# orybkin/video-gcp

Hardware: AMD Instinct MI355X
Metric: predicted frames/sec, 64x64x3 seq_len=80 gcp_tree (posterior forward + all loss terms, model(inputs) and model.loss() of train.py:157-159, batch-stat BatchNorm) (higher is better)
Workload: dtype f32 (encoder / decoder convs and the tree GEMMs from 512 rows: split-f16 MFMA with f32 accumulate, f32-equivalent; everything else exact f32 MFMA)

## Files before the change

### video-gcp_amd/csrc/conv3x3_split.hip

```cpp
#include "common.h"
#include "split_mfma.h"

#include <cstdlib>
#include <type_traits>

namespace {

struct SplitUpCfg {
    static constexpr int RW = 18, RH = 6, LW = 10, LH = 4, CC = 16, KS = 5;
    static constexpr int RAW_BYTES = LH * LW * CC * 4;
    static constexpr int PLANE_BYTES = RH * RW * 32;
    static constexpr int WAVE_BYTES = RAW_BYTES + 2 * PLANE_BYTES;
    static constexpr int NS = (LH * LW * 4 + 63) / 64;
    static constexpr int W_CHUNK_BYTES = KS * 2 * 1024;
    static int lds_bytes(int nchunk) { return nchunk * W_CHUNK_BYTES + 8 * WAVE_BYTES + 8 * 2 * 16 * 4; }
};

__global__ void __launch_bounds__(512, 2) conv3x3_up16_split_kernel(const gcpx_conv_args a, const int items_per_wave,
                                                                    const int nitems) {
    using Cfg = SplitUpCfg;
    constexpr int RW = Cfg::RW, RH = Cfg::RH, LW = Cfg::LW, LH = Cfg::LH, CC = Cfg::CC, NS = Cfg::NS, KS = Cfg::KS;
    extern __shared__ float4 smem4[];
    const int nchunk = a.Cin / CC;
    const char* wl = reinterpret_cast<const char*>(smem4);
// ... 798 lines not shown
    __syncthreads();

    const int c4 = lane & 3, ps = lane >> 2;
    const float* sptr = a.src[0].ptr;
    const int srcC = a.src[0].C;
    float4 bn_s = make_float4(1.f, 1.f, 1.f, 1.f), bn_t = make_float4(0.f, 0.f, 0.f, 0.f);
    if (a.src[0].scale) {
        bn_s = *reinterpret_cast<const float4*>(a.src[0].scale + c4 * 4);
        bn_t = *reinterpret_cast<const float4*>(a.src[0].shift + c4 * 4);
    }
    const float slope = a.src[0].act == GCPX_ACT_LRELU ? 0.2f : 1.f;
    const int fdiv0 = a.src[0].frame_div;
    const int ew = a.w_split_log2_dev ? __builtin_amdgcn_readfirstlane(*a.w_split_log2_dev) : a.w_split_log2;
    const float4 bv = *reinterpret_cast<const float4*>(a.bias + q * 4);

    const int gw = blockIdx.x * 8 + wave;
    int item = gw * items_per_wave;
    const int item_end = min(item + items_per_wave, nitems);
    auto origin = [&](int it, int& f, int& y0, int& x0) {
        const int rb = it % nrb;
        const int t = it / nrb;
        y0 = rb * R; f = t / ncb; x0 = (t % ncb) * 16;
    };
    int p_row[NS], p_col[NS], p_lds[NS];
    bool p_ok[NS];
#pragma unroll
    for (int k = 0; k < NS; ++k) {
        const int pix = ps + 16 * k;
        p_ok[k] = pix < PR * PW;
        p_row[k] = min(pix, PR * PW - 1) / PW;
        p_col[k] = min(pix, PR * PW - 1) % PW;
        p_lds[k] = (p_row[k] * PW + p_col[k]) * 64 + c4 * 16;
    }
    int r_rd[NO], r_wr[NO];
    float r_wa[NO];
    bool r_ok[NO], r_c0[NO], r_c17[NO];
#pragma unroll
    for (int k = 0; k < NO; ++k) {
        const int pix = ps + 16 * k;
        r_ok[k] = pix < PR * RW;
        const int r = min(pix, PR * RW - 1) / RW, c = min(pix, PR * RW - 1) % RW;
        r_rd[k] = (r * PW + (c >> 1)) * 64 + c4 * 16;
        r_wr[k] = (r * RW + c) * 32 + c4 * 8;
        r_wa[k] = (c & 1) ? 0.25f : 0.75f;
        r_c0[k] = c == 0; r_c17[k] = c == RW - 1;
    }
    float4 pre[NS];
    auto issue_loads = [&](int it) {
        int f, y0, x0;
        origin(it, f, y0, x0);
        const float* base = sptr + (size_t)(f / fdiv0) * Hin * Win * srcC + c4 * 4;
        const int ly0 = y0 - 1, lx0 = x0 / 2 - 1;
#pragma unroll
        for (int k = 0; k < NS; ++k) {
            const int sy = min(max(ly0 + p_row[k], 0), Hin - 1), sx = min(max(lx0 + p_col[k], 0), Win - 1);
            pre[k] = *reinterpret_cast<const float4*>(base + (unsigned)((sy * Win + sx) * srcC));
        }
    };

    f32x4 st1 = f32x4{0, 0, 0, 0}, st2 = f32x4{0, 0, 0, 0};
    f32x4 outv[R][2];
    float* optr = nullptr;
    auto store_out = [&]() __attribute__((always_inline)) {
#pragma unroll
        for (int yi = 0; yi < R; ++yi)
#pragma unroll
            for (int py = 0; py < 2; ++py) {
                const f32x4 v = outv[yi][py];
                *reinterpret_cast<float4*>(optr + (unsigned)((2 * yi + py) * W * 16)) = make_float4(v[0], v[1], v[2], v[3]);
            }
    };
    if (item < item_end) issue_loads(item);

    const int boff0 = (j + (q >> 1)) * 32 + (q & 1) * 16, boff1 = (j + 2) * 32 + (q & 1) * 16;

    for (; item < item_end; ++item) {
        int f, y0, x0;
        origin(item, f, y0, x0);
        const bool top = (y0 == 0), bot = (y0 + R == Hin), lft = (x0 == 0), rgt = (x0 + 16 == W);

        float amax = 0.f;
#pragma unroll
        for (int k = 0; k < NS; ++k) {
            float4 v = pre[k];
            v.x = fmaf(v.x, bn_s.x, bn_t.x); v.y = fmaf(v.y, bn_s.y, bn_t.y); v.z = fmaf(v.z, bn_s.z, bn_t.z); v.w = fmaf(v.w, bn_s.w, bn_t.w);
            v.x = fmaxf(v.x, v.x * slope); v.y = fmaxf(v.y, v.y * slope); v.z = fmaxf(v.z, v.z * slope); v.w = fmaxf(v.w, v.w * slope);
            if (p_ok[k]) *reinterpret_cast<float4*>(wbuf + p_lds[k]) = v;
            else v = make_float4(0.f, 0.f, 0.f, 0.f);
            amax = fmaxf(amax, fmaxf(fmaxf(fabsf(v.x), fabsf(v.y)), fmaxf(fabsf(v.z), fabsf(v.w))));
        }
        if (item + 1 < item_end) issue_loads(item + 1);
        if (optr) store_out();
        amax = wave_max_nonneg(amax);
        int ex = 14 + 127 - (int)((__float_as_uint(amax) >> 23) & 0xff);
        ex = __builtin_amdgcn_readfirstlane(amax > 0.f ? max(-100, min(min(100, 126 - ew), ex)) : min(100, 126 - ew));
        const float sx2 = __uint_as_float((unsigned)(127 + ex) << 23);

        h4 o1[NO], o2[NO];
#pragma unroll
        for (int k = 0; k < NO; ++k) {
            const float4 A = *reinterpret_cast<const float4*>(wbuf + r_rd[k]);
            const float4 B = *reinterpret_cast<const float4*>(wbuf + r_rd[k] + 64);
            const float sc = ((lft && r_c0[k]) || (rgt && r_c17[k])) ? 0.f : sx2;
            const float wa = r_wa[k] * sc, wb = (1.f - r_wa[k]) * sc;
            float4 v;
            v.x = fmaf(wa, A.x, wb * B.x); v.y = fmaf(wa, A.y, wb * B.y); v.z = fmaf(wa, A.z, wb * B.z); v.w = fmaf(wa, A.w, wb * B.w);
            h4 p1, p2;
            p1[0] = (_Float16)v.x; p1[1] = (_Float16)v.y; p1[2] = (_Float16)v.z; p1[3] = (_Float16)v.w;
            p2[0] = (_Float16)fmaf((float)p1[0], -1.f, v.x); p2[1] = (_Float16)fmaf((float)p1[1], -1.f, v.y);
            p2[2] = (_Float16)fmaf((float)p1[2], -1.f, v.z); p2[3] = (_Float16)fmaf((float)p1[3], -1.f, v.w);
            o1[k] = p1;
            o2[k] = p2;
        }
        __builtin_amdgcn_fence(__ATOMIC_ACQ_REL, "wavefront");
        __builtin_amdgcn_wave_barrier();
#pragma unroll
        for (int k = 0; k < NO; ++k) {
            if (r_ok[k]) {
                *reinterpret_cast<h4*>(wbuf + r_wr[k]) = o1[k];
                *reinterpret_cast<h4*>(wbuf + r_wr[k] + Cfg::PLANE_BYTES) = o2[k];
            }
        }

        f32x4 acc[R][2];
#pragma unroll
        for (int yi = 0; yi < R; ++yi) { acc[yi][0] = f32x4{0, 0, 0, 0}; acc[yi][1] = f32x4{0, 0, 0, 0}; }
        auto load_w = [&](const int t, h8 (&w)[2]) __attribute__((always_inline)) {
            const char* wp = wl + t * 2048 + lane * 16;
            w[0] = *reinterpret_cast<const h8*>(wp);
            w[1] = *reinterpret_cast<const h8*>(wp + 1024);
        };
        auto load_b = [&](const int kind, const int r, h8 (&b)[2]) __attribute__((always_inline)) {
            const char* bp = wbuf + r * RW * 32 + (kind ? boff1 : boff0);
            b[0] = *reinterpret_cast<const h8*>(bp);
            b[1] = *reinterpret_cast<const h8*>(bp + Cfg::PLANE_BYTES);
        };
        h8 wq[2][2], bq[2][PR][2], wt[2], wb[2];
        load_w(0, wq[0]);
#pragma unroll
        for (int r = 0; r < 4; ++r) load_b(0, r, bq[0][r]);
        __builtin_amdgcn_s_setprio(1);
        static_for<0, 12>([&](auto tc) __attribute__((always_inline)) {
            constexpr int t = decltype(tc)::value, kind = t / 6, blk = t % 6, dyl = blk / 2, py = blk % 2;
// ... 14 lines not shown
#pragma unroll
            for (int yi = 0; yi < R; ++yi) acc[yi][py] = mfma32h(w1, bq[kind & 1][yi + dyl][1], acc[yi][py]);
#pragma unroll
            for (int yi = 0; yi < R; ++yi) acc[yi][py] = mfma32h(w1, bq[kind & 1][yi + dyl][0], acc[yi][py]);
            __builtin_amdgcn_sched_group_barrier(0x100, (more ? 2 : 0) + ((pre_next || pre_own) ? 2 : 0) + (pre_c ? 4 : 0), 0);
            __builtin_amdgcn_sched_group_barrier(0x008, 12, 0);
            if constexpr (blk == 5) {
                if (top) {
                    acc[0][0] = mfma32h(wt[1], bq[kind & 1][0][0], acc[0][0]);
                    acc[0][0] = mfma32h(wt[0], bq[kind & 1][0][1], acc[0][0]);
                    acc[0][0] = mfma32h(wt[0], bq[kind & 1][0][0], acc[0][0]);
                }
                if (bot) {
                    acc[R - 1][1] = mfma32h(wb[1], bq[kind & 1][PR - 1][0], acc[R - 1][1]);
                    acc[R - 1][1] = mfma32h(wb[0], bq[kind & 1][PR - 1][1], acc[R - 1][1]);
                    acc[R - 1][1] = mfma32h(wb[0], bq[kind & 1][PR - 1][0], acc[R - 1][1]);
                }
            }
        });
        __builtin_amdgcn_s_setprio(0);

        const float inv = __uint_as_float((unsigned)(127 - ex - ew) << 23);
        optr = a.out + (((size_t)f * H + 2 * y0) * W + x0 + j) * 16 + q * 4;
        const float* adp = a.addend ? a.addend + (((size_t)(f / a.addend_frame_div) * H + 2 * y0) * W + x0 + j) * 16 + q * 4 : nullptr;
#pragma unroll
        for (int yi = 0; yi < R; ++yi)
#pragma unroll
            for (int py = 0; py < 2; ++py) {
                f32x4 v = acc[yi][py];
                v[0] = fmaf(v[0], inv, bv.x); v[1] = fmaf(v[1], inv, bv.y); v[2] = fmaf(v[2], inv, bv.z); v[3] = fmaf(v[3], inv, bv.w);
                if (adp) {
                    const float4 ad = *reinterpret_cast<const float4*>(adp + (unsigned)((2 * yi + py) * W * 16));
                    v[0] += ad.x; v[1] += ad.y; v[2] += ad.z; v[3] += ad.w;
                }
                outv[yi][py] = v;
                st1 += v;
                st2 += v * v;
            }
    }
    if (optr) store_out();
    if (a.stats_partial) {
#pragma unroll
        for (int r = 0; r < 4; ++r) {
            const float s1 = row16_sum(st1[r]);
            const float s2 = row16_sum(st2[r]);
            if (j == 0) {
                red[(wave * 2 + 0) * 16 + q * 4 + r] = s1;
                red[(wave * 2 + 1) * 16 + q * 4 + r] = s2;
            }
        }
        __syncthreads();
        if (tid < 32) {
            const int which = tid >> 4, c = tid & 15;
            float sum = 0.f;
#pragma unroll
// ... 443 lines not shown
```

### video-gcp_amd/forward_plan.py

```python
import ctypes as C
import os
from contextlib import contextmanager

import torch

from . import packing as pk
from . import runtime as rt
from .hparams import GCPHParams
from .params import init_params, encoder_layers, encoder_skip_layers, decoder_layers
from .plan_ops import _Plan, _addr, N_LANES


class ForwardPlanMixin:

    def _plan_encoder(self, plan, tag, x_ptr, F, out_ptr, out_ob, out_orow, out_rpb):
        hp, P, lib = self._hp, self.pk, self.lib
        G = lib.gcpx_conv4x4s2_grid()
        S = hp.img_sz
        skip_idx = encoder_skip_layers(hp)
        skips = {}
        a0 = self._buf(f"{tag}.a0", (F, S // 2, S // 2, hp.ngf))
        enc_rec = dict(F=F, x_ptr=x_ptr, a0=a0, r={}, out=(out_ptr, out_ob, out_orow, out_rpb))
        plan.rec[f"enc:{tag}"] = enc_rec
        plan.add(f"enc.input:{tag}", lib.gcpx_conv4x4s2_image, x_ptr, P["enc.input.w"].data_ptr(),
# ... 47 lines not shown
        T, nz, dk = hp.max_seq_len, hp.nz_enc, hp.nz_attn_key
        li = l if hp.untied_layers else 0
        qin = self._buf(f"attn.qin{l}", (M, dk))
        self._mlp(plan, f"attn.query{l}", W["attn.query"], [el, er], M, n, out=qin.data_ptr(), ob=n * dk, orow=dk)
        dense = lambda t, w: self._rowsrc(t.data_ptr(), 0, w, w)
        qp = self._buf(f"attn.q{l}", (M, dk))
        self._gemm(plan, f"attn.q_proj{l}", [dense(qin, dk)], M, dk, M, W["attn.q_proj.w"], W["attn.q_proj.b"],
                   out=qp.data_ptr(), ob=0, orow=dk)
        o = self._buf(f"attn.o{l}", (M, nz))
        gamma = self._buf(f"attn.gamma{l}", (M, T))
        temp = self.sd[f"tree_module.tree_modules.{li}.inference.attention.attention_layers.0.temperature"]
        plan.add(f"attn{l}", lib.gcpx_attention, qp.data_ptr(), _addr(Kp, li * B * T * dk), _addr(Vp, li * B * T * nz), None,
                 tin["end_ind"].data_ptr(), temp.data_ptr(), o.data_ptr(), gamma.data_ptr(), M, n, T, dk, nz, hp.n_attention_heads)
        raw = self._buf(f"attn.raw{l}", (M, nz))
        self._gemm(plan, f"attn.out_proj{l}", [dense(o, nz)], M, nz, M, W["attn.out_proj.w"], W["attn.out_proj.b"],
                   out=raw.data_ptr(), ob=0, orow=nz)
        et = self._buf(f"attn.e_tilde{l}", (M, nz))
        self._gemm(plan, f"attn.out{l}", [dense(raw, nz)], M, nz, M, W["attn.out.w"], W["attn.out.b"], out=et.data_ptr(), ob=0, orow=nz)
        plan.rec.setdefault("gamma", {})[l] = gamma
        plan.rec.setdefault("e_tilde", {})[l] = et
        plan.rec.setdefault("attn", {})[l] = dict(qin=qin, qp=qp, o=o, raw=raw, gamma=gamma, et=et, M=M, n=n, li=li, temp=temp)
        return self._rowsrc(et.data_ptr(), n * nz, nz, nz)

    def _plan_decoder_features(self, plan, e_src, F, rpb, skips):
        hp, P, lib = self._hp, self.pk, self.lib
        ctop = self._c_top
        d0 = self._buf("dec.d0", (F, 4, 4, ctop))
        plan.rec["dec"] = dict(F=F, rpb=rpb, e_src=e_src, d0=d0, blocks=[], skips=skips)
        nrb = lib.gcpx_gemm_row_blocks(F, 16 * ctop)
        st = self._buf("dec.st0", (nrb, 2, 16 * ctop)) if self.training else None
        self._gemm(plan, "dec.input", [e_src], F, 16 * ctop, rpb, P["dec.input.w"], P["dec.input.b"], out=d0.data_ptr(),
                   ob=rpb * 16 * ctop, orow=16 * ctop, stats=st)
        sc, sh = self._bn(plan, "dec.bn0", "decoder.net.input.norm", ctop, st, nrb, 16 * ctop, F * 16)
        prev = (d0.data_ptr(), ctop, 1, sc, sh, rt.ACT_LRELU)
        res = 4
        for name, c_prev, c_skip, skip_idx, cout in decoder_layers(hp):
            srcs = [prev]
            if skip_idx >= 0:
                t, C_, ssc, ssh, sact = skips[skip_idx]
                assert C_ == c_skip and t.shape[1] == res
                srcs.append((t.data_ptr(), C_, rpb, ssc, ssh, sact))
            o = self._buf(f"dec.{name}", (F, 2 * res, 2 * res, cout))
            cpad = (cout + 15) // 16 * 16
            hoist = (skip_idx >= 0 and rpb > 1 and F % rpb == 0 and self.split_f16 and cout in (32, 64) and c_prev % 32 == 0 and
                     c_skip % 32 == 0 and f"dec.{name}" in self.pk_split and "fold" not in self.pk_split[f"dec.{name}"] and
                     os.environ.get("GCPX_NO_SKIP_HOIST") is None)
            hoist16 = (skip_idx >= 0 and rpb > 1 and F % rpb == 0 and self.split_f16 and cout == 16 and c_prev == 16 and c_skip == 16 and
                       f"dec.{name}.f16a" in self.pk_split and res % 4 == 0 and os.environ.get("GCPX_SKIP_HOIST16") == "1")
            addend = None
            if hoist16:
                addend = self._buf(f"dec.{name}.skip", (F // rpb, 2 * res, 2 * res, cout))
                t, C_, ssc, ssh, sact = skips[skip_idx]
                zb = self._buf(f"dec.{name}.zero_bias", (cpad,), zero=True)
                a_s = self._conv_args([(t.data_ptr(), C_, 1, ssc, ssh, sact)], F // rpb, res, res, 2 * res, 2 * res, cout, cout,
                                      P[f"dec.{name}.w"], zb, addend, upsample=1)
                self._set_split(a_s, f"dec.{name}.f16b")
                plan.keep.append(a_s)
                plan.add(f"dec.{name}.skip", lib.gcpx_conv3x3, C.byref(a_s))
                srcs_main = [prev]
            elif hoist:
                addend = self._buf(f"dec.{name}.skip", (F // rpb, 2 * res, 2 * res, cout))
                t, C_, ssc, ssh, sact = skips[skip_idx]
                zb = self._buf(f"dec.{name}.zero_bias", (cpad,), zero=True)
                a_s = self._conv_args([(t.data_ptr(), C_, 1, ssc, ssh, sact)], F // rpb, res, res, 2 * res, 2 * res, cout, cout,
                                      P[f"dec.{name}.w"], zb, addend, upsample=1)
                self._set_split(a_s, f"dec.{name}")
                a_s.wpk_split = a_s.wpk_split + (c_prev // 32) * 9 * (cpad // 16) * 2048
                plan.keep.append(a_s)
                plan.add(f"dec.{name}.skip", lib.gcpx_conv3x3, C.byref(a_s))
                srcs_main = [prev]
            else:
                srcs_main = srcs
            a = self._conv_args(srcs_main, F, res, res, 2 * res, 2 * res, cout, cout, P[f"dec.{name}.w"], P[f"dec.{name}.b"],
                                o, upsample=1, stats=(o if self.training else None))
            if hoist or hoist16:
                a.addend, a.addend_frame_div = addend.data_ptr(), rpb
            self._set_split(a, f"dec.{name}.f16a" if hoist16 else f"dec.{name}")
            Gl = lib.gcpx_conv3x3_grid(C.byref(a))
            assert Gl > 0, rt.lib().gcpx_last_error()
            st = self._buf(f"dec.st.{name}", (Gl, 2, cpad)) if self.training else None
            a.stats_partial = st.data_ptr() if st is not None else None
            plan.keep.append(a)
            plan.add(f"dec.{name}", lib.gcpx_conv3x3, C.byref(a))
            plan.rec["dec"]["blocks"].append(dict(name=name, srcs=srcs, out=o, res_in=res, cout=cout, c_prev=c_prev, c_skip=c_skip,
                                                  skip_idx=skip_idx))
            res *= 2
            sc, sh = self._bn(plan, f"dec.bn.{name}", f"decoder.net.{name}.norm", cout, st, Gl, cpad, F * res * res)
            prev = (o.data_ptr(), cout, 1, sc, sh, rt.ACT_LRELU)
        assert res == hp.img_sz
        return prev

    def _build_plan(self, key, tin):
        hp, P, lib = self._hp, self.pk, self.lib
        B, has_traj, has_z, sample_prior, phase = key[0], key[1], key[2], key[3], key[4]
        pred_len = key[9]
        train_aux = has_traj and phase == "train" and not sample_prior
        L, T, N = hp.hierarchy_levels, hp.max_seq_len, hp.n_nodes
        nz, nv, H, SD = hp.nz_enc, hp.nz_vae, hp.nz_mid_lstm, hp.lstm_state_dim
        PS = 2 ** L + 1
        plan = _Plan(lib)
# ... 56 lines not shown
                    else:
                        kenc = self._buf("inf_key_enc", (B * T, nz))
                        self._plan_seq_encoder(plan, "kseq", "inf_key_encoder.0", enc_traj, kenc, B)
                    keys = self._buf("inf_enc_key_seq", (B * T, dk))
                    dense = lambda t, w: self._rowsrc(t.data_ptr(), 0, w, w)
                    self._gemm(plan, "kseq.key", [dense(kenc, nz)], B * T, dk, B * T, P["kseq.key.w"], P["kseq.key.b"],
                               out=keys.data_ptr(), ob=0, orow=dk)
                    Kp = self._buf("attn.K", (n_mod, B * T, dk))
                    Vp = self._buf("attn.V", (n_mod, B * T, nz))
                    self._gemm(plan, "attn.k_proj", [dense(keys, dk)], B * T, dk, B * T, P["attn.k_proj.w"], P["attn.k_proj.b"],
                               out=Kp.data_ptr(), ob=0, orow=dk, batch=(n_mod, 0, P["attn.k_proj.w"][0].numel(), dk, B * T * dk))
                    self._gemm(plan, "attn.v_proj", [dense(inf_enc, nz)], B * T, nz, B * T, P["attn.v_proj.w"], P["attn.v_proj.b"],
                               out=Vp.data_ptr(), ob=0, orow=nz, batch=(n_mod, 0, P["attn.v_proj.w"][0].numel(), nz, B * T * nz))
                    plan.rec["attn_kv"] = dict(Kp=Kp, Vp=Vp, keys=keys, kenc=kenc, n_mod=n_mod)

        if traj_first:
            plan_traj_encoder()
        plan.lane = 1
        if "rng_all" in tin:
            plan.add("randn", lib.gcpx_randn, tin["rng_all"].data_ptr(), tin["rng_all"].numel(), self._buf("rng_state", (2,), torch.int64).data_ptr())
            if "aux_n" in tin and not pred_len:
                plan.wait(2, 1)
        skips = self._plan_encoder(plan, "I0", tin["I_0"].data_ptr(), B, _addr(E), PS * nz, 0, 1)
        plan.lane = 2
        if not pred_len:
            if "aux_n" in tin:
                plan_aux_indices()
            plan_bookkeeping()
        if hp.attach_cost_mdl and hp.run_cost_mdl and train_aux and self._has_aux_training:
            gt = self._buf("cost_target", (B,))
            rows = hp.input_nc * hp.img_sz
            plan.add("path_cost", lib.gcpx_path_cost, tin["traj_seq"].data_ptr(), tin["cost_start_idx"].data_ptr(),
                     tin["cost_end_idx"].data_ptr(), B, T, rows, hp.img_sz, self._buf("cost_partial", (B, rows)).data_ptr(), gt.data_ptr())
        self._plan_encoder(plan, "Ig", tin["I_g"].data_ptr(), B, _addr(E, 2 ** L * nz), PS * nz, 0, 1)
        outs = {}
        e0 = lambda: self._rowsrc(_addr(E), PS * nz, 0, nz)
        eg = lambda: self._rowsrc(_addr(E, 2 ** L * nz), PS * nz, 0, nz)
        if hp.regress_length and not pred_len:
            plan.wait(2, 1)
            logits = self._buf("seq_len_logits", (B, T))
            self._mlp(plan, "length_pred", P["length_pred"], [e0(), eg()], B, 1, out=logits.data_ptr(), ob=T, orow=0)
            outs["seq_len_logits"] = logits
        if not traj_first:
            plan_traj_encoder()
        plan.lane = 0
        plan.join([1, 2])
# ... 191 lines not shown
            la.seq_len = seq_len.data_ptr()
            if "actions_sampled" in outs and "actions" in tin:
                la.action_pred, la.action_seq, la.inv_t0 = outs["actions_sampled"].data_ptr(), tin["actions"].data_ptr(), tin["inv_t0"].data_ptr()
                la.n_actions, la.w_action = hp.n_actions, hp.action_rec_weight
            if "cost_pred" in outs:
                la.cost_pred, la.cost_target, la.w_cost = outs["cost_pred"].data_ptr(), outs["cost_target"].data_ptr(), 1.0
            loss_out = self._buf("losses", (16,), zero=True)
            la.out, la.B, la.T, la.N, la.state_dim = loss_out.data_ptr(), B, T, (N - 1 if adaptive else N), hp.state_dim
            la.w_rec, la.w_kl, la.w_len, la.w_exist, la.w_state = hp.dense_img_rec_weight, hp.kl_weight, hp.length_pred_weight, 1.0, 1.0
            if self._kl_w is not None:
                la.w_kl_dev = self._kl_w.data_ptr()
            la.total_div = float(T * hp.input_nc * hp.img_sz * hp.img_sz)
            plan.keep.append(la)
            return la, kl_b

        decode, with_loss = key[8], key[7]
        loss_pre = None
        if with_loss and not adaptive:
            loss_pre = loss_args()
            plan.add("loss.pre", lib.gcpx_loss_pre, C.byref(loss_pre[0]), *kl_args(loss_pre[1]))
        if decode:
            F = B * N
            S = hp.img_sz
            prev = self._plan_decoder_features(plan, self._rowsrc(_addr(E, nz), PS * nz, nz, nz), F, N, skips)
            images = self._buf("images_df", (B, N, hp.input_nc, S, S))
            distr = matched_distr = None
            with_loss = key[7]
            dlm = hp.decoder_distribution == "discrete_logistic_mixture"
            head_out, row_map = None, None
            fused_nll = None
            if dlm:
                mode = rt.HEAD_DLM_MEAN
                if self.materialize_distr or (adaptive and self.save_for_backward and with_loss):
                    mode, distr = rt.HEAD_DLM_BOTH, self._buf("distr_df", (B, N, S, S, self._head_pitch))
                    head_out = distr
                elif self._head_grad_fused(key):
                    mode, row_map = rt.HEAD_DLM_NLL_GRAD, node2row
                    head_out = self._buf("bw.dMD", (B * T, S, S, self._head_pitch))
                    fused_nll = self._buf("nll_partial", ((S // 4) * (S // 16), B * T), zero=True)
                    plan.rec["nll_bwd_fused"] = plan.rec["head_grad_fused"] = True
                elif with_loss and not adaptive and not self.save_for_backward and self._head_nll_fusable():
                    mode, row_map = rt.HEAD_DLM_NLL, node2row
                    fused_nll = self._buf("nll_partial", ((S // 4) * (S // 16), B * T), zero=True)
                elif with_loss and not adaptive:
                    mode, matched_distr = rt.HEAD_DLM_BOTH, self._buf("matched_distr", (B, T, S, S, self._head_pitch))
                    head_out, row_map = matched_distr, node2row
            else:
# ... 123 lines not shown
```

### video-gcp_amd/model.py

```python
import ctypes as C
import os
from contextlib import contextmanager

import torch

from . import packing as pk
from . import runtime as rt
from .hparams import GCPHParams
from .params import init_params, encoder_layers, encoder_skip_layers, decoder_layers
from .plan_ops import _Plan, Outputs, ModelOutputs, PlanOpsMixin, _addr, N_LANES
from .weights import WeightsMixin
from .forward_plan import ForwardPlanMixin
from .replay import ReplayMixin


class GCPTreeModel(WeightsMixin, PlanOpsMixin, ForwardPlanMixin, ReplayMixin):

    _has_aux_training = True
    _has_pred_length = True
    _rng_in_plan = True

    _n_models = 0
    _stream_pool = {}

# ... 23 lines not shown
        GCPTreeModel._n_models += 1
        self.n_steps = 0
        self._kl_w = None
        self.use_graph = {"graph": True, "eager": False}.get(os.environ.get("GCPX_FORWARD_REPLAY", "auto"), "auto")
        pool_key = (self.device.index, os.environ.get("GCPX_MAIN_PRIORITY", "0"))
        pool = None if os.environ.get("GCPX_PRIVATE_STREAMS") else GCPTreeModel._stream_pool.get(pool_key)
        if pool is None:
            main = torch.cuda.Stream(device=self.device, priority=int(os.environ.get("GCPX_MAIN_PRIORITY", "0")))
            lanes = [main.cuda_stream]
            for _ in range(N_LANES - 1):
                sp = C.c_void_p()
                with torch.cuda.device(self.device):
                    rt.check(self.lib.gcpx_stream_create(C.byref(sp)), "stream_create")
                lanes.append(sp)
            pool = (main, lanes)
            if not os.environ.get("GCPX_PRIVATE_STREAMS"):
                GCPTreeModel._stream_pool[pool_key] = pool
        self._stream, self._streams = pool[0], list(pool[1])
        self._set_kl_weight()
        self.save_for_backward = False
        self.split_f16 = os.environ.get("GCPX_EXACT_F32") is None
        self.fused_head_nll = os.environ.get("GCPX_UNFUSED_NLL") is None
        self.head32 = os.environ.get("GCPX_HEAD32", "0") == "1"
        self._timed_op = None
        self._timed_events = []
        self._pack_all()
        from . import handles as Hd
        self.encoder, self.decoder, self.dense_rec = Hd.EncoderHandle(self), Hd.DecoderHandle(self), Hd.DenseRecHandle(self)
        self.tree_module = Hd.TreeModuleHandle(self)
        if hp.attach_inv_mdl:
            self.inv_mdl = Hd.InverseModelHandle(self)
        if hp.attach_cost_mdl:
            self.cost_mdl = Hd.CostModelHandle(self)

    def _check_hp(self, hp):
        assert hp.matching_type in ("balanced", "dtw_image")
        if hp.tree_lstm not in ("split_linear", "linear", "sum", ""):
            raise ValueError("don't know this TreeLSTM type")
        if hp.seq_enc not in ("conv", "none"):
            raise ValueError(f"seq_enc = {hp.seq_enc!r}: 'conv' (ConvSeqEncodingModule) and 'none' (Identity) are built")
        if hp.lstm_init not in ("mlp", "zero"):
            raise ValueError("dont know lstm init type {}!".format(hp.lstm_init))
        if hp.attentive_inference:
            assert hp.n_attention_layers == 1, "one attention layer is built (hyperparameters.py:25 default)"
        assert not (hp.action_conditioned_pred or hp.deterministic or hp.non_goal_conditioned), \
            "the vmpc.py variants belong to the flat predictor (SequentialModel): GCPSequentialModel"
# ... 329 lines not shown
```

### video-gcp_amd/sequential.py

```python
import ctypes as C

import torch

from . import runtime as rt
from .model import GCPTreeModel, Outputs, _Plan, _addr
from .params import init_params_sequential


class GCPSequentialModel(GCPTreeModel):
    _has_aux_training = True
    _has_pred_length = False
    _rng_in_plan = False
    _has_training = True

    def _check_hp(self, hp):
        assert hp.lstm_init in ("zero", "mlp")
        assert hp.n_actions <= 16 or not hp.action_conditioned_pred, "the action rows are padded to one 16-column k-group"

    @property
    def _nets(self):
        return ("gen_lstm",) if self._hp.deterministic else ("prior_lstm", "inf_lstm", "gen_lstm")

    def _default_params(self, hp, seed):
        return init_params_sequential(hp, seed)
# ... 130 lines not shown
        hp, P, lib = self._hp, self.pk, self.lib
        B, has_traj, has_z, sample_prior, phase, with_loss = key[0], key[1], key[2], key[3], key[4], key[7]
        T, nz, nv, H, nl = hp.max_seq_len, hp.nz_enc, hp.nz_vae, hp.nz_mid_lstm, hp.n_lstm_layers
        S = hp.img_sz
        plan = _Plan(lib)
        X = self._buf("seq.X", (B, T, nz))
        EG = self._buf("seq.EG", (B, nz))
        PZ = self._buf("seq.PZ", (B, T - 1, 2 * nv))
        QZ = self._buf("seq.QZ", (B, T - 1, 2 * nv), zero=True)
        Z = self._buf("seq.Z", (B, T - 1, nv))
        idx = self._buf("seq.idx", (B, T), torch.int32)
        seq_len = self._buf("seq.len", (B,), torch.int32)
        plan.add("seq_index", lib.gcpx_seq_index, tin["end_ind"].data_ptr(), B, T, idx.data_ptr(), seq_len.data_ptr())
        train_aux = has_traj and phase == "train" and not sample_prior
        if "aux_n" in tin:
            AUXK = ("inv_t0", "inv_t1", "cost_start_idx", "cost_end_idx")
            plan.add("aux_sample_indices", lib.gcpx_aux_sample_indices_gauss, tin["end_ind"].data_ptr(), tin["aux_n"].data_ptr(), B,
                     hp.inv_mdl_temp_dist, *[tin[k].data_ptr() for k in AUXK])

        enc_traj = None
        plan.fork([1, 2])
        plan.lane = 1
        skips = self._plan_encoder(plan, "I0", tin["I_0"].data_ptr(), B, _addr(X), T * nz, 0, 1)
        plan.lane = 2
        if hp.attach_cost_mdl and hp.run_cost_mdl and train_aux and "cost_start_idx" in tin:
            rows = hp.input_nc * hp.img_sz
            plan.add("path_cost", lib.gcpx_path_cost, tin["traj_seq"].data_ptr(), tin["cost_start_idx"].data_ptr(),
                     tin["cost_end_idx"].data_ptr(), B, T, rows, hp.img_sz, self._buf("cost_partial", (B, rows)).data_ptr(),
                     self._buf("cost_target", (B,)).data_ptr())
        self._plan_encoder(plan, "Ig", tin["I_g"].data_ptr(), B, _addr(EG), nz, 0, 1)
        plan.lane = 0
        if has_traj:
            enc_traj = self._buf("enc_traj", (B * T, nz))
            self._plan_encoder(plan, "traj", tin["traj_seq"].data_ptr(), B * T, enc_traj.data_ptr(), T * nz, nz, T)
        plan.join([1, 2])
        outs = {}
        e0 = lambda: self._rowsrc(_addr(X), T * nz, 0, nz)
        eg = lambda: self._rowsrc(_addr(EG), nz, 0, nz)
        if hp.regress_length:
            logits = self._buf("seq_len_logits", (B, T))
            self._mlp(plan, "length_pred", P["length_pred"], [e0(), eg()], B, 1, out=logits.data_ptr(), ob=T, orow=0)
            outs["seq_len_logits"] = logits

        EA = None
        if hp.action_conditioned_pred:
            na = hp.n_actions
# ... 174 lines not shown
            first = enc_traj if has_traj else mes
            s0 = self._rowsrc(first.data_ptr(), T * nz, nz, nz)
            s1 = self._rowsrc(_addr(mes, nz), T * nz, nz, nz)
            self._mlp(plan, "inv_mdl", P["inv_mdl"], [s0, s1], B * (T - 1), T - 1, out=act.data_ptr(),
                      ob=(T - 1) * hp.n_actions, orow=hp.n_actions)
            outs["actions_padded"] = act
        if aux_ok and ((hp.attach_inv_mdl and not hp.train_inv_mdl_full_seq) or (hp.attach_cost_mdl and hp.run_cost_mdl)):
            aux_rows = self._buf("aux_rows", (4, B), torch.int32)
            plan.add("aux_index_rows", lib.gcpx_aux_index_rows, tin["inv_t0"].data_ptr(), tin["inv_t1"].data_ptr(),
                     tin["cost_start_idx"].data_ptr(), tin["cost_end_idx"].data_ptr(), B, T, T, aux_rows.data_ptr())
            gather = lambda t, i: self._rowsrc(t.data_ptr(), 0, nz, nz, rowidx=aux_rows[i])
            if hp.attach_inv_mdl and not hp.train_inv_mdl_full_seq:
                act = self._buf("actions_sampled", (B, hp.n_actions))
                self._mlp(plan, "inv_mdl", P["inv_mdl"], [gather(enc_traj, 0), gather(mes, 1)], B, B, out=act.data_ptr(), ob=0,
                          orow=hp.n_actions)
                outs["actions_sampled"] = act
            if hp.attach_cost_mdl and hp.run_cost_mdl:
                cost = self._buf("cost_pred", (B, 1))
                self._mlp(plan, "cost_mdl", P["cost_mdl"], [gather(mes, 2), gather(mes, 3)], B, B, out=cost.data_ptr(), ob=0, orow=1)
                outs["cost_pred"], outs["cost_target"] = cost, self._buf("cost_target", (B,))
        plan.lane = 0

        F = B * (T - 1)
        prev = self._plan_decoder_features(plan, self._rowsrc(_addr(X, nz), T * nz, nz, nz), F, T - 1, skips)
        dec_images = self._buf("seq.dec_images", (B, T - 1, hp.input_nc, S, S))
        dlm = hp.decoder_distribution == "discrete_logistic_mixture"
        head_out = row_map = matched = fused_nll = None
        if dlm:
            mode = rt.HEAD_DLM_MEAN
            if with_loss or self.materialize_distr:
                row_map = self._buf("seq.row_map", (F,), torch.int32)
                row_map.copy_((torch.arange(B)[:, None] * T + torch.arange(1, T)[None]).reshape(-1).to(torch.int32))
                if with_loss and self._head_nll_fusable():
                    fused_nll = self._buf("nll_partial", ((S // 4) * (S // 16), B * T), zero=True)
                    mode = rt.HEAD_DLM_NLL
                    if self.save_for_backward:
                        mode, head_out = rt.HEAD_DLM_NLL_GRAD, self._buf("bw.dMD", (B * T, S, S, self._head_pitch))
                        r2f = self._buf("seq.row2frame", (B * T,), torch.int32)
                        inv = torch.arange(B * T, dtype=torch.int64).view(B, T) // T * (T - 1) + torch.arange(T)[None] - 1
                        inv[:, 0] = -1
                        r2f.copy_(inv.reshape(-1).to(torch.int32))
                        plan.add("zero_unmapped", lib.gcpx_zero_unmapped_rows, head_out.data_ptr(), S * S * self._head_pitch,
                                 r2f.data_ptr(), B * T)
                        plan.rec["nll_bwd_fused"] = plan.rec["head_grad_fused"] = True
                else:
                    mode, matched = rt.HEAD_DLM_BOTH, self._buf("matched_distr", (B, T, S, S, self._head_pitch))
                    head_out = matched
# ... 123 lines not shown
```

### video-gcp_amd/weights.py

```python
import ctypes as C
import os
from contextlib import contextmanager

import torch

from . import packing as pk
from . import runtime as rt
from .hparams import GCPHParams
from .params import init_params, encoder_layers, encoder_skip_layers, decoder_layers
from .plan_ops import _addr


class WeightsMixin:

    def _flatten_params(self, params):
        off, self._poff = 0, {}
        for k, v in params.items():
            self._poff[k] = (off, tuple(v.shape))
            off += (v.numel() + 3) // 4 * 4
        self.theta = torch.zeros(off, dtype=torch.float32, device=self.device)
        self.sd = {}
        for k, v in params.items():
            o, shp = self._poff[k]
            view = self.theta[o:o + v.numel()].view(shp)
# ... 23 lines not shown
        d["b_out"] = pk.pad_vec(sd[f"{prefix}.head.linear.bias"], out_pad)
        return d

    def _pack_all(self):
        if self._arena is not None:
            self.repack()
            return
        self.pk = self._pack_tree(self.sd)
        if self._hp.tree_lstm:
            self._pack_fused_embed()
        self._pack_split()
        self._pack_gemm_split()

    def _pack_split(self):
        self.pk_split = {}
        hp = self._hp
        todo = []
        if hp.decoder_distribution == "discrete_logistic_mixture":
            todo.append(("dec.head", "decoder.gen_head.conv.weight", pk.dlm_channel_perm(hp.n_mixtures)))
            if self.head32 and hp.n_mixtures == 10 and hp.head_channels == 100:
                todo.append(("dec.head32", "decoder.gen_head.conv.weight", ("head32", pk.dlm_channel_perm(hp.n_mixtures))))
        for name, c_prev, c_skip, skip_idx, cout in decoder_layers(hp):
            if cout == 16 and c_prev + c_skip == 32:
                todo.append((f"dec.{name}", f"decoder.net.{name}.conv.weight", "rowfold"))
            elif cout == 16:
                todo.append((f"dec.{name}", f"decoder.net.{name}.conv.weight", None))
            elif cout in (32, 64) and (c_prev + c_skip) % 32 == 0:
                todo.append((f"dec.{name}", f"decoder.net.{name}.conv.weight", "tiled32"))
        for name, cin, cout, norm in self._enc_layers[1:]:
            if cin == 16 or cin % 32 == 0:
                todo.append((f"enc.{name}", f"encoder.net.{name}.conv.weight", "enc4x4"))
        for name, key, perm in todo:
            off, shp = self._poff[key]
            d = {}
            if perm == "enc4x4":
                idx = pk.conv4x4_split_index(shp, off).to(self.device)
            elif perm == "rowfold":
                d["fold"] = torch.zeros(24 * shp[0] * shp[1], dtype=torch.float32, device=self.device)
                d["fold_src"] = (off, shp[0], shp[1])
                idx = pk.conv3x3_fold_index().to(self.device)
            elif perm == "tiled32":
                idx = pk.conv3x3_split32_index(shp, off).to(self.device)
            elif isinstance(perm, tuple) and perm[0] == "head32":
                idx = pk.head32_index(shp, off, perm[1]).to(self.device)
            else:
                idx = pk.conv3x3_split_index(shp, off, perm).to(self.device)
            d.update(idx=idx, out=torch.zeros(2 * idx.numel(), dtype=torch.int16, device=self.device),
                     log2=torch.zeros(1, dtype=torch.int32, device=self.device))
            self.pk_split[name] = d
            if perm == "rowfold" and shp[1] == 32:
                for tag, cbase in (("f16a", 0), ("f16b", 16)):
                    i16 = pk.conv3x3_fold16_index(shp[1], cbase).to(self.device)
                    self.pk_split[f"{name}.{tag}"] = dict(fold=d["fold"], fold16=True, idx=i16,
                                                          out=torch.zeros(2 * i16.numel(), dtype=torch.int16, device=self.device),
                                                          log2=torch.zeros(1, dtype=torch.int32, device=self.device))
        self.repack_split()

    def repack_split(self, stream=None):
        st = stream if stream is not None else torch.cuda.current_stream(self.device).cuda_stream
        if not self.pk_split:
            return
        tab = self._split_tab
        key = (self.theta.data_ptr(),) + tuple((d["out"].data_ptr(), d["idx"].data_ptr()) for d in self.pk_split.values())
        if tab is None or tab[2] != key:
            descs = []
            for name, d in self.pk_split.items():
                src = d["fold"] if "fold" in d else self.theta
                e = rt.SplitPackDesc()
                e.src, e.idx, e.out, e.log2_out, e.n = src.data_ptr(), d["idx"].data_ptr(), d["out"].data_ptr(), d["log2"].data_ptr(), d["idx"].numel()
                descs.append(e)
            arr = (rt.SplitPackDesc * len(descs))(*descs)
            dev = torch.frombuffer(bytearray(bytes(arr)), dtype=torch.uint8).to(self.device)
            tab = self._split_tab = (dev, len(descs), key, torch.zeros(len(descs), dtype=torch.int32, device=self.device))
        for name, d in self.pk_split.items():
            if "fold_src" in d:
                off, cout, cin = d["fold_src"]
                rt.check(self.lib.gcpx_fold_upsample_weights(self.theta.data_ptr() + 4 * off, cout, cin, d["fold"].data_ptr(), st), "fold_upsample_weights")
        rt.check(self.lib.gcpx_split_pack_group2(tab[0].data_ptr(), tab[1], tab[3].data_ptr(), st), "split_pack_group2")

# ... 263 lines not shown
```

Baseline: 500,800.

## Hoist decoder skip-half convs to encoder lane and recompute per-lane indices in upsample kernel

The decoder's skip-connection half-convolutions are now planned right after the encoder on the parallel lane, so they can overlap other work instead of sitting on the decoder's critical path. In the upsample split kernel, per-lane index arrays are dropped and recomputed on the fly to reduce register pressure. The addend loads are also issued early, before the MFMA loop, to hide their latency. This adds code paths for a fold16 packing variant, but that variant stays behind an environment flag, and the scheduling change introduces a cross-lane dependency on the skip buffers.

```diff
diff --git a/video-gcp_amd/csrc/conv3x3_split.hip b/video-gcp_amd/csrc/conv3x3_split.hip
--- a/video-gcp_amd/csrc/conv3x3_split.hip
+++ b/video-gcp_amd/csrc/conv3x3_split.hip
@@ -844,38 +844,16 @@
         const int t = it / nrb;
         y0 = rb * R; f = t / ncb; x0 = (t % ncb) * 16;
     };
-    int p_row[NS], p_col[NS], p_lds[NS];
-    bool p_ok[NS];
-#pragma unroll
-    for (int k = 0; k < NS; ++k) {
-        const int pix = ps + 16 * k;
-        p_ok[k] = pix < PR * PW;
-        p_row[k] = min(pix, PR * PW - 1) / PW;
-        p_col[k] = min(pix, PR * PW - 1) % PW;
-        p_lds[k] = (p_row[k] * PW + p_col[k]) * 64 + c4 * 16;
-    }
-    int r_rd[NO], r_wr[NO];
-    float r_wa[NO];
-    bool r_ok[NO], r_c0[NO], r_c17[NO];
-#pragma unroll
-    for (int k = 0; k < NO; ++k) {
-        const int pix = ps + 16 * k;
-        r_ok[k] = pix < PR * RW;
-        const int r = min(pix, PR * RW - 1) / RW, c = min(pix, PR * RW - 1) % RW;
-        r_rd[k] = (r * PW + (c >> 1)) * 64 + c4 * 16;
-        r_wr[k] = (r * RW + c) * 32 + c4 * 8;
-        r_wa[k] = (c & 1) ? 0.25f : 0.75f;
-        r_c0[k] = c == 0; r_c17[k] = c == RW - 1;
-    }
     float4 pre[NS];
-    auto issue_loads = [&](int it) {
+    auto issue_loads = [&](int it, int psv) {
         int f, y0, x0;
         origin(it, f, y0, x0);
         const float* base = sptr + (size_t)(f / fdiv0) * Hin * Win * srcC + c4 * 4;
         const int ly0 = y0 - 1, lx0 = x0 / 2 - 1;
 #pragma unroll
         for (int k = 0; k < NS; ++k) {
-            const int sy = min(max(ly0 + p_row[k], 0), Hin - 1), sx = min(max(lx0 + p_col[k], 0), Win - 1);
+            const int pix = min(psv + 16 * k, PR * PW - 1), p_row = pix / PW, p_col = pix % PW;
+            const int sy = min(max(ly0 + p_row, 0), Hin - 1), sx = min(max(lx0 + p_col, 0), Win - 1);
             pre[k] = *reinterpret_cast<const float4*>(base + (unsigned)((sy * Win + sx) * srcC));
         }
     };
@@ -883,6 +861,8 @@
     f32x4 st1 = f32x4{0, 0, 0, 0}, st2 = f32x4{0, 0, 0, 0};
     f32x4 outv[R][2];
     float* optr = nullptr;
+    float4 adv[R][2];
+    const bool has_addend = a.addend != nullptr;
     auto store_out = [&]() __attribute__((always_inline)) {
 #pragma unroll
         for (int yi = 0; yi < R; ++yi)
@@ -892,7 +872,7 @@
                 *reinterpret_cast<float4*>(optr + (unsigned)((2 * yi + py) * W * 16)) = make_float4(v[0], v[1], v[2], v[3]);
             }
     };
-    if (item < item_end) issue_loads(item);
+    if (item < item_end) issue_loads(item, ps);
 
     const int boff0 = (j + (q >> 1)) * 32 + (q & 1) * 16, boff1 = (j + 2) * 32 + (q & 1) * 16;
 
@@ -900,6 +880,9 @@
         int f, y0, x0;
         origin(item, f, y0, x0);
         const bool top = (y0 == 0), bot = (y0 + R == Hin), lft = (x0 == 0), rgt = (x0 + 16 == W);
+        int psv = ps;
+        asm volatile("" : "+v"(psv));
+        psv &= 15;
 
         float amax = 0.f;
 #pragma unroll
@@ -907,11 +890,19 @@
             float4 v = pre[k];
             v.x = fmaf(v.x, bn_s.x, bn_t.x); v.y = fmaf(v.y, bn_s.y, bn_t.y); v.z = fmaf(v.z, bn_s.z, bn_t.z); v.w = fmaf(v.w, bn_s.w, bn_t.w);
             v.x = fmaxf(v.x, v.x * slope); v.y = fmaxf(v.y, v.y * slope); v.z = fmaxf(v.z, v.z * slope); v.w = fmaxf(v.w, v.w * slope);
-            if (p_ok[k]) *reinterpret_cast<float4*>(wbuf + p_lds[k]) = v;
+            const int pix = psv + 16 * k;
+            if (pix < PR * PW) *reinterpret_cast<float4*>(wbuf + pix * 64 + c4 * 16) = v;
             else v = make_float4(0.f, 0.f, 0.f, 0.f);
             amax = fmaxf(amax, fmaxf(fmaxf(fabsf(v.x), fabsf(v.y)), fmaxf(fabsf(v.z), fabsf(v.w))));
         }
-        if (item + 1 < item_end) issue_loads(item + 1);
+        if (item + 1 < item_end) issue_loads(item + 1, psv);
+        if (has_addend) {
+            const float* adp = a.addend + (((size_t)(f / a.addend_frame_div) * H + 2 * y0) * W + x0 + j) * 16 + q * 4;
+#pragma unroll
+            for (int yi = 0; yi < R; ++yi)
+#pragma unroll
+                for (int py = 0; py < 2; ++py) adv[yi][py] = *reinterpret_cast<const float4*>(adp + (unsigned)((2 * yi + py) * W * 16));
+        }
         if (optr) store_out();
         amax = wave_max_nonneg(amax);
         int ex = 14 + 127 - (int)((__float_as_uint(amax) >> 23) & 0xff);
@@ -921,10 +912,13 @@
         h4 o1[NO], o2[NO];
 #pragma unroll
         for (int k = 0; k < NO; ++k) {
-            const float4 A = *reinterpret_cast<const float4*>(wbuf + r_rd[k]);
-            const float4 B = *reinterpret_cast<const float4*>(wbuf + r_rd[k] + 64);
-            const float sc = ((lft && r_c0[k]) || (rgt && r_c17[k])) ? 0.f : sx2;
-            const float wa = r_wa[k] * sc, wb = (1.f - r_wa[k]) * sc;
+            const int pix = min(psv + 16 * k, PR * RW - 1), r = pix / RW, c = pix % RW;
+            const int r_rd = (r * PW + (c >> 1)) * 64 + c4 * 16;
+            const float r_wa = (c & 1) ? 0.25f : 0.75f;
+            const float4 A = *reinterpret_cast<const float4*>(wbuf + r_rd);
+            const float4 B = *reinterpret_cast<const float4*>(wbuf + r_rd + 64);
+            const float sc = ((lft && c == 0) || (rgt && c == RW - 1)) ? 0.f : sx2;
+            const float wa = r_wa * sc, wb = (1.f - r_wa) * sc;
             float4 v;
             v.x = fmaf(wa, A.x, wb * B.x); v.y = fmaf(wa, A.y, wb * B.y); v.z = fmaf(wa, A.z, wb * B.z); v.w = fmaf(wa, A.w, wb * B.w);
             h4 p1, p2;
@@ -938,9 +932,10 @@
         __builtin_amdgcn_wave_barrier();
 #pragma unroll
         for (int k = 0; k < NO; ++k) {
-            if (r_ok[k]) {
-                *reinterpret_cast<h4*>(wbuf + r_wr[k]) = o1[k];
-                *reinterpret_cast<h4*>(wbuf + r_wr[k] + Cfg::PLANE_BYTES) = o2[k];
+            const int pix = psv + 16 * k;
+            if (pix < PR * RW) {
+                *reinterpret_cast<h4*>(wbuf + pix * 32 + c4 * 8) = o1[k];
+                *reinterpret_cast<h4*>(wbuf + pix * 32 + c4 * 8 + Cfg::PLANE_BYTES) = o2[k];
             }
         }
 
@@ -1001,15 +996,14 @@
 
         const float inv = __uint_as_float((unsigned)(127 - ex - ew) << 23);
         optr = a.out + (((size_t)f * H + 2 * y0) * W + x0 + j) * 16 + q * 4;
-        const float* adp = a.addend ? a.addend + (((size_t)(f / a.addend_frame_div) * H + 2 * y0) * W + x0 + j) * 16 + q * 4 : nullptr;
 #pragma unroll
         for (int yi = 0; yi < R; ++yi)
 #pragma unroll
             for (int py = 0; py < 2; ++py) {
                 f32x4 v = acc[yi][py];
                 v[0] = fmaf(v[0], inv, bv.x); v[1] = fmaf(v[1], inv, bv.y); v[2] = fmaf(v[2], inv, bv.z); v[3] = fmaf(v[3], inv, bv.w);
-                if (adp) {
-                    const float4 ad = *reinterpret_cast<const float4*>(adp + (unsigned)((2 * yi + py) * W * 16));
+                if (has_addend) {
+                    const float4 ad = adv[yi][py];
                     v[0] += ad.x; v[1] += ad.y; v[2] += ad.z; v[3] += ad.w;
                 }
                 outv[yi][py] = v;
diff --git a/video-gcp_amd/forward_plan.py b/video-gcp_amd/forward_plan.py
--- a/video-gcp_amd/forward_plan.py
+++ b/video-gcp_amd/forward_plan.py
@@ -93,7 +93,44 @@
         plan.rec.setdefault("attn", {})[l] = dict(qin=qin, qp=qp, o=o, raw=raw, gamma=gamma, et=et, M=M, n=n, li=li, temp=temp)
         return self._rowsrc(et.data_ptr(), n * nz, nz, nz)
 
-    def _plan_decoder_features(self, plan, e_src, F, rpb, skips):
+    def _skip_hoist_kind(self, name, c_prev, c_skip, skip_idx, cout, res, F, rpb):
+        if not (skip_idx >= 0 and rpb > 1 and F % rpb == 0 and self.split_f16) or os.environ.get("GCPX_NO_SKIP_HOIST") is not None:
+            return None
+        if (cout in (32, 64) and c_prev % 32 == 0 and c_skip % 32 == 0 and f"dec.{name}" in self.pk_split and
+                "fold" not in self.pk_split[f"dec.{name}"]):
+            return "tiled"
+        if (cout == 16 and c_prev == 16 and c_skip == 16 and self._skip_hoist16 and f"dec.{name}.f16a" in self.pk_split and res % 4 == 0):
+            return "fold16"
+        return None
+
+    def _plan_skip_half(self, plan, kind, name, c_prev, cout, res, F, rpb, skip):
+        P, lib = self.pk, self.lib
+        cpad = (cout + 15) // 16 * 16
+        addend = self._buf(f"dec.{name}.skip", (F // rpb, 2 * res, 2 * res, cout))
+        t, C_, ssc, ssh, sact = skip
+        zb = self._buf(f"dec.{name}.zero_bias", (cpad,), zero=True)
+        a_s = self._conv_args([(t.data_ptr(), C_, 1, ssc, ssh, sact)], F // rpb, res, res, 2 * res, 2 * res, cout, cout,
+                              P[f"dec.{name}.w"], zb, addend, upsample=1)
+        if kind == "fold16":
+            self._set_split(a_s, f"dec.{name}.f16b")
+        else:
+            self._set_split(a_s, f"dec.{name}")
+            a_s.wpk_split = a_s.wpk_split + (c_prev // 32) * 9 * (cpad // 16) * 2048
+        plan.keep.append(a_s)
+        plan.add(f"dec.{name}.skip", lib.gcpx_conv3x3, C.byref(a_s))
+        return addend
+
+    def _plan_decoder_skips(self, plan, F, rpb, skips):
+        addends = {}
+        res = 4
+        for name, c_prev, c_skip, skip_idx, cout in decoder_layers(self._hp):
+            kind = self._skip_hoist_kind(name, c_prev, c_skip, skip_idx, cout, res, F, rpb)
+            if kind:
+                addends[name] = self._plan_skip_half(plan, kind, name, c_prev, cout, res, F, rpb, skips[skip_idx])
+            res *= 2
+        return addends
+
+    def _plan_decoder_features(self, plan, e_src, F, rpb, skips, addends=None):
         hp, P, lib = self._hp, self.pk, self.lib
         ctop = self._c_top
         d0 = self._buf("dec.d0", (F, 4, 4, ctop))
@@ -113,40 +150,21 @@
                 srcs.append((t.data_ptr(), C_, rpb, ssc, ssh, sact))
             o = self._buf(f"dec.{name}", (F, 2 * res, 2 * res, cout))
             cpad = (cout + 15) // 16 * 16
-            hoist = (skip_idx >= 0 and rpb > 1 and F % rpb == 0 and self.split_f16 and cout in (32, 64) and c_prev % 32 == 0 and
-                     c_skip % 32 == 0 and f"dec.{name}" in self.pk_split and "fold" not in self.pk_split[f"dec.{name}"] and
-                     os.environ.get("GCPX_NO_SKIP_HOIST") is None)
-            hoist16 = (skip_idx >= 0 and rpb > 1 and F % rpb == 0 and self.split_f16 and cout == 16 and c_prev == 16 and c_skip == 16 and
-                       f"dec.{name}.f16a" in self.pk_split and res % 4 == 0 and os.environ.get("GCPX_SKIP_HOIST16") == "1")
+            kind = self._skip_hoist_kind(name, c_prev, c_skip, skip_idx, cout, res, F, rpb)
             addend = None
-            if hoist16:
-                addend = self._buf(f"dec.{name}.skip", (F // rpb, 2 * res, 2 * res, cout))
-                t, C_, ssc, ssh, sact = skips[skip_idx]
-                zb = self._buf(f"dec.{name}.zero_bias", (cpad,), zero=True)
-                a_s = self._conv_args([(t.data_ptr(), C_, 1, ssc, ssh, sact)], F // rpb, res, res, 2 * res, 2 * res, cout, cout,
-                                      P[f"dec.{name}.w"], zb, addend, upsample=1)
-                self._set_split(a_s, f"dec.{name}.f16b")
-                plan.keep.append(a_s)
-                plan.add(f"dec.{name}.skip", lib.gcpx_conv3x3, C.byref(a_s))
-                srcs_main = [prev]
-            elif hoist:
-                addend = self._buf(f"dec.{name}.skip", (F // rpb, 2 * res, 2 * res, cout))
-                t, C_, ssc, ssh, sact = skips[skip_idx]
-                zb = self._buf(f"dec.{name}.zero_bias", (cpad,), zero=True)
-                a_s = self._conv_args([(t.data_ptr(), C_, 1, ssc, ssh, sact)], F // rpb, res, res, 2 * res, 2 * res, cout, cout,
-                                      P[f"dec.{name}.w"], zb, addend, upsample=1)
-                self._set_split(a_s, f"dec.{name}")
-                a_s.wpk_split = a_s.wpk_split + (c_prev // 32) * 9 * (cpad // 16) * 2048
-                plan.keep.append(a_s)
-                plan.add(f"dec.{name}.skip", lib.gcpx_conv3x3, C.byref(a_s))
-                srcs_main = [prev]
+            if kind:
+                addend = addends[name] if addends is not None else self._plan_skip_half(plan, kind, name, c_prev, cout, res, F, rpb,
+                                                                                         skips[skip_idx])
+            a = self._conv_args([prev] if kind else srcs, F, res, res, 2 * res, 2 * res, cout, cout, P[f"dec.{name}.w"], P[f"dec.{name}.b"],
+                                o, upsample=1, stats=(o if self.training else None))
+            if kind:
+                a.addend, a.addend_frame_div = addend.data_ptr(), rpb
+            if kind == "fold16":
+                self._set_split(a, f"dec.{name}.f16a")
+            elif f"dec.{name}.f16a" in self.pk_split:
+                self._set_split(a, self._split_pack_fold32(name))
             else:
-                srcs_main = srcs
-            a = self._conv_args(srcs_main, F, res, res, 2 * res, 2 * res, cout, cout, P[f"dec.{name}.w"], P[f"dec.{name}.b"],
-                                o, upsample=1, stats=(o if self.training else None))
-            if hoist or hoist16:
-                a.addend, a.addend_frame_div = addend.data_ptr(), rpb
-            self._set_split(a, f"dec.{name}.f16a" if hoist16 else f"dec.{name}")
+                self._set_split(a, f"dec.{name}")
             Gl = lib.gcpx_conv3x3_grid(C.byref(a))
             assert Gl > 0, rt.lib().gcpx_last_error()
             st = self._buf(f"dec.st.{name}", (Gl, 2, cpad)) if self.training else None
@@ -249,6 +267,7 @@
             if "aux_n" in tin and not pred_len:
                 plan.wait(2, 1)
         skips = self._plan_encoder(plan, "I0", tin["I_0"].data_ptr(), B, _addr(E), PS * nz, 0, 1)
+        dec_addends = self._plan_decoder_skips(plan, B * N, N, skips) if key[8] else None
         plan.lane = 2
         if not pred_len:
             if "aux_n" in tin:
@@ -486,7 +505,7 @@
         if decode:
             F = B * N
             S = hp.img_sz
-            prev = self._plan_decoder_features(plan, self._rowsrc(_addr(E, nz), PS * nz, nz, nz), F, N, skips)
+            prev = self._plan_decoder_features(plan, self._rowsrc(_addr(E, nz), PS * nz, nz, nz), F, N, skips, dec_addends)
             images = self._buf("images_df", (B, N, hp.input_nc, S, S))
             distr = matched_distr = None
             with_loss = key[7]
diff --git a/video-gcp_amd/model.py b/video-gcp_amd/model.py
--- a/video-gcp_amd/model.py
+++ b/video-gcp_amd/model.py
@@ -69,6 +69,7 @@
         self.split_f16 = os.environ.get("GCPX_EXACT_F32") is None
         self.fused_head_nll = os.environ.get("GCPX_UNFUSED_NLL") is None
         self.head32 = os.environ.get("GCPX_HEAD32", "0") == "1"
+        self._skip_hoist16 = os.environ.get("GCPX_SKIP_HOIST16") == "1" and os.environ.get("GCPX_NO_SKIP_HOIST") is None
         self._timed_op = None
         self._timed_events = []
         self._pack_all()
diff --git a/video-gcp_amd/sequential.py b/video-gcp_amd/sequential.py
--- a/video-gcp_amd/sequential.py
+++ b/video-gcp_amd/sequential.py
@@ -176,6 +176,7 @@
         plan.fork([1, 2])
         plan.lane = 1
         skips = self._plan_encoder(plan, "I0", tin["I_0"].data_ptr(), B, _addr(X), T * nz, 0, 1)
+        dec_addends = self._plan_decoder_skips(plan, B * (T - 1), T - 1, skips)
         plan.lane = 2
         if hp.attach_cost_mdl and hp.run_cost_mdl and train_aux and "cost_start_idx" in tin:
             rows = hp.input_nc * hp.img_sz
@@ -396,7 +397,7 @@
         plan.lane = 0
 
         F = B * (T - 1)
-        prev = self._plan_decoder_features(plan, self._rowsrc(_addr(X, nz), T * nz, nz, nz), F, T - 1, skips)
+        prev = self._plan_decoder_features(plan, self._rowsrc(_addr(X, nz), T * nz, nz, nz), F, T - 1, skips, dec_addends)
         dec_images = self._buf("seq.dec_images", (B, T - 1, hp.input_nc, S, S))
         dlm = hp.decoder_distribution == "discrete_logistic_mixture"
         head_out = row_map = matched = fused_nll = None
diff --git a/video-gcp_amd/weights.py b/video-gcp_amd/weights.py
--- a/video-gcp_amd/weights.py
+++ b/video-gcp_amd/weights.py
@@ -69,7 +69,10 @@
                 todo.append(("dec.head32", "decoder.gen_head.conv.weight", ("head32", pk.dlm_channel_perm(hp.n_mixtures))))
         for name, c_prev, c_skip, skip_idx, cout in decoder_layers(hp):
             if cout == 16 and c_prev + c_skip == 32:
-                todo.append((f"dec.{name}", f"decoder.net.{name}.conv.weight", "rowfold"))
+                if self._skip_hoist16 and self.split_f16 and skip_idx >= 0 and c_prev == 16 and c_skip == 16:
+                    todo.append((f"dec.{name}", f"decoder.net.{name}.conv.weight", "rowfold16"))
+                else:
+                    todo.append((f"dec.{name}", f"decoder.net.{name}.conv.weight", "rowfold"))
             elif cout == 16:
                 todo.append((f"dec.{name}", f"decoder.net.{name}.conv.weight", None))
             elif cout in (32, 64) and (c_prev + c_skip) % 32 == 0:
@@ -78,30 +81,46 @@
             if cin == 16 or cin % 32 == 0:
                 todo.append((f"enc.{name}", f"encoder.net.{name}.conv.weight", "enc4x4"))
         for name, key, perm in todo:
-            off, shp = self._poff[key]
-            d = {}
-            if perm == "enc4x4":
-                idx = pk.conv4x4_split_index(shp, off).to(self.device)
-            elif perm == "rowfold":
+            self._add_split_pack(name, key, perm)
+        self.repack_split()
+
+    def _add_split_pack(self, name, key, perm):
+        off, shp = self._poff[key]
+        d = {}
+        if perm == "rowfold16":
+            fold = torch.zeros(24 * shp[0] * shp[1], dtype=torch.float32, device=self.device)
+            for tag, cbase in (("f16a", 0), ("f16b", 16)):
+                i16 = pk.conv3x3_fold16_index(shp[1], cbase).to(self.device)
+                self.pk_split[f"{name}.{tag}"] = dict(fold=fold, fold16=True, idx=i16,
+                                                      out=torch.zeros(2 * i16.numel(), dtype=torch.int16, device=self.device),
+                                                      log2=torch.zeros(1, dtype=torch.int32, device=self.device))
+            self.pk_split[f"{name}.f16a"]["fold_src"] = (off, shp[0], shp[1])
+            return
+        if perm == "enc4x4":
+            idx = pk.conv4x4_split_index(shp, off).to(self.device)
+        elif perm == "rowfold":
+            shared = self.pk_split.get(f"{name}.f16a")
+            if shared is not None:
+                d["fold"] = shared["fold"]
+            else:
                 d["fold"] = torch.zeros(24 * shp[0] * shp[1], dtype=torch.float32, device=self.device)
                 d["fold_src"] = (off, shp[0], shp[1])
-                idx = pk.conv3x3_fold_index().to(self.device)
-            elif perm == "tiled32":
-                idx = pk.conv3x3_split32_index(shp, off).to(self.device)
-            elif isinstance(perm, tuple) and perm[0] == "head32":
-                idx = pk.head32_index(shp, off, perm[1]).to(self.device)
-            else:
-                idx = pk.conv3x3_split_index(shp, off, perm).to(self.device)
-            d.update(idx=idx, out=torch.zeros(2 * idx.numel(), dtype=torch.int16, device=self.device),
-                     log2=torch.zeros(1, dtype=torch.int32, device=self.device))
-            self.pk_split[name] = d
-            if perm == "rowfold" and shp[1] == 32:
-                for tag, cbase in (("f16a", 0), ("f16b", 16)):
-                    i16 = pk.conv3x3_fold16_index(shp[1], cbase).to(self.device)
-                    self.pk_split[f"{name}.{tag}"] = dict(fold=d["fold"], fold16=True, idx=i16,
-                                                          out=torch.zeros(2 * i16.numel(), dtype=torch.int16, device=self.device),
-                                                          log2=torch.zeros(1, dtype=torch.int32, device=self.device))
-        self.repack_split()
+            idx = pk.conv3x3_fold_index().to(self.device)
+        elif perm == "tiled32":
+            idx = pk.conv3x3_split32_index(shp, off).to(self.device)
+        elif isinstance(perm, tuple) and perm[0] == "head32":
+            idx = pk.head32_index(shp, off, perm[1]).to(self.device)
+        else:
+            idx = pk.conv3x3_split_index(shp, off, perm).to(self.device)
+        d.update(idx=idx, out=torch.zeros(2 * idx.numel(), dtype=torch.int16, device=self.device),
+                 log2=torch.zeros(1, dtype=torch.int32, device=self.device))
+        self.pk_split[name] = d
+
+    def _split_pack_fold32(self, name):
+        if f"dec.{name}" not in self.pk_split:
+            self._add_split_pack(f"dec.{name}", f"decoder.net.{name}.conv.weight", "rowfold")
+            self.repack_split()
+        return f"dec.{name}"
 
     def repack_split(self, stream=None):
         st = stream if stream is not None else torch.cuda.current_stream(self.device).cuda_stream
```

Result: no change. 505,400 (median of 6 runs) (+0.9%).
